# dachinzo/ringpop-node

Measured on AMD Instinct MI355X. Metric: ring lookups/s + member-updates merged/s; SWIM round time @100k members, higher is better.
Workload: dtype u32; 1 GPU; C2: 10000-server HashRing x 100 replica points, batched lookupN(n=3) of 36-byte keys, 2^26 keys per step; servers=10000, replica_points=100, total_keys=164550934528, parallelism=keys sharded, ring replicated

## Files before the change

ringpop-node_amd/csrc/rp_ring.hip:

```cpp
#include <algorithm>
#include <chrono>
#include <cstdio>
#include <cstdlib>
#include <cstring>
#include <memory>
#include <mutex>
#include <string>
#include <unordered_map>
#include <vector>

#include "../../include/ringpop_amd.h"
#include "rp_farmhash.h"
#include "rp_philox.h"
#include "rp_hashlong.h"
#include "rp_names.h"
#include "rp_prims.h"

namespace rp {

constexpr uint32_t NIL = 0xFFFFFFFFu;

static bool getenv_flag(const char* name) {
    const char* v = getenv(name);
    return v && *v && *v != '0';
// ... 620 lines not shown

#ifdef RP_LK_PROF
__device__ unsigned long long g_lk_prof[10];
#define LK_T(var, dep) \
    uint64_t var;      \
    asm volatile("s_memtime %0\n\ts_waitcnt lgkmcnt(0)" : "=s"(var) : "v"(dep))
#else
#define LK_T(var, dep)
#endif

#ifdef RP_LK_ABLATE
#define RP_LKA(cv) ((cv).ablate)
#else
#define RP_LKA(cv) 0u
#endif
template <int KPL, int NEED, int HS = 1, bool FUSE = false, int STG = 0, int LH = 1>
__global__ __launch_bounds__(kLkThreads) __attribute__((amdgpu_waves_per_eu(4))) void k_lookupn_lean(const uint8_t* __restrict__ keys, uint64_t ntiles,
                                                             CompactView cv, uint32_t* __restrict__ out,
                                                             uint8_t* __restrict__ counts,
                                                             uint32_t* __restrict__ slow_list,
                                                             uint32_t* __restrict__ slow_cnt, CompactFixView fv,
                                                             int np) {
    constexpr int LEN = 36, W4 = LEN / 4;
    constexpr int TK = kLkThreads * KPL;
    constexpr int V4 = TK * W4 / 4;
    constexpr int PER = (V4 + kLkThreads - 1) / kLkThreads;
    constexpr int NW = kLkThreads / 64;
    constexpr uint32_t SPAN = 5 - NEED;
    static_assert((TK * W4) % 4 == 0 && (TK * NEED) % 4 == 0 && NEED >= 1 && NEED <= 4, "tile shape");
    static_assert(KPL % HS == 0 && V4 % HS == 0, "slices of whole keys");
    constexpr int SK = TK * W4 / HS, SO = TK * NEED;
    constexpr int VS = V4 / HS;
    constexpr int SKR = STG ? 2 * SK : SK;
    static_assert(STG == 0 || (SK * 4) % 1024 == 0, "DMA slices of whole 1-KB wave pieces");
    __shared__ __attribute__((aligned(16))) uint32_t lds[SKR > SO ? SKR : SO];
    constexpr uint32_t AG = 64;
    __shared__ uint32_t ag[NW][3][AG];
    __shared__ uint32_t nslow_tile;
    uint32_t* const sk = lds;
    uint32_t* const so = lds;
    const int tid = threadIdx.x, lane = tid & 63, wv = tid >> 6;
    const uint32_t omask = (1u << cv.ob) - 1u, obit = 1u << cv.ob;
    const uint32_t bsh = 32u - cv.cb;
    const uint32_t rmask = (1u << bsh) - 1u;
    const __amdgpu_buffer_rsrc_t ent_r =
        __builtin_amdgcn_make_buffer_rsrc(const_cast<uint8_t*>(cv.ent), 0, (int)cv.ent_bytes, 0x00020000);
    const bool hinted = NEED == 3 && cv.idxh != nullptr && !(RP_LKA(cv) & 4u);
    const __amdgpu_buffer_rsrc_t idx_r = __builtin_amdgcn_make_buffer_rsrc(
        const_cast<uint32_t*>(hinted ? cv.idxh : cv.idx), 0, (int)cv.idx_bytes, 0x00020000);
    auto load16 = [&](uint32_t pos) {
        return __builtin_bit_cast(u32x4, __builtin_amdgcn_raw_buffer_load_b128(ent_r, (int)(3u * pos), 0, 0));
    };
    auto ent5v = [&](const u32x4 v, uint32_t (&e)[5]) {
        e[0] = v.x & 0xFFFFFFu;
        e[1] = (v.x >> 24) | ((v.y & 0xFFFFu) << 8);
        e[2] = (v.y >> 16) | ((v.z & 0xFFu) << 16);
        e[3] = v.z >> 8;
        e[4] = v.w & 0xFFFFFFu;
    };
    auto wstart = [&](uint32_t hk, uint32_t bck, uint32_t hint) -> uint32_t {
        const int fl = (int)((((hk << cv.cb) >> 24) * bck) >> 8) - 2 + (int)hint;
        return (NEED >= 2 && cv.wpred && bck <= 10u && fl > 0) ? (uint32_t)fl : 0u;
    };
    auto finish2 = [&](const u32x4 win, uint32_t K, uint32_t w2, uint32_t* row, uint8_t* cnt, uint32_t* nsl,
                       uint32_t* slist) {
        const uint32_t kk = w2 & 0xFFFu, bck = (w2 >> 12) & 15u, b0 = (w2 >> 17) & 15u;
        uint32_t e2[5];
        ent5v(win, e2);
        uint32_t off = 0;
        bool slow = false;
        if ((w2 >> 16) & 1u) {
            bool tie = false;
#pragma unroll
            for (int j = 0; j < 5; j++) {
                const bool inb = (uint32_t)j + b0 < bck;
                off += (inb && e2[j] < K);
                tie |= (inb && e2[j] - K < obit);
            }
            slow = (tie && !cv.exact) | (off == 5u && bck > b0 + 5u) | (((w2 >> 21) & 1u) && off == 0u);
        }
        uint32_t res[4] = {NIL, NIL, NIL, NIL};
        const uint32_t rc = dedupe5(e2, off, omask, NEED, res);
        slow |= rc < (uint32_t)NEED;
        if (slow) {
            const uint32_t sp = atomicAdd(nsl, 1u);
            if (sp < kSlowPerTile) slist[sp] = kk;
        }
#pragma unroll
        for (int q = 0; q < NEED; q++) row[kk * NEED + q] = res[q];
        if (cnt) cnt[kk] = (uint8_t)rc;
    };
#ifdef RP_LK_PROF
    uint64_t pa[6] = {0, 0, 0, 0, 0, 0}, ntl = 0;
#endif
    for (uint64_t t = blockIdx.x; t < ntiles; t += gridDim.x) {
        const uint64_t base = t * TK;
        uint32_t h[KPL];
        LK_T(t0, tid);
        if constexpr (STG == 1 || STG == 2) {
            constexpr int SLB = SK * 4, SLI = SLB / 1024, PW = SLI / NW, PX = SLI % NW;
            const uint8_t* src = keys + base * LEN;
            uint8_t* ring = reinterpret_cast<uint8_t*>(lds);
            auto dma = [&](int sl) {
#pragma unroll
                for (int i = 0; i < PW + 1; i++)
                    if (i < PW || wv < PX) {
// ... 40 lines not shown
#pragma unroll
                for (int k = hs * (KPL / HS); k < (hs + 1) * (KPL / HS); k++) {
                    uint32_t w[W4];
#pragma unroll
                    for (int j = 0; j < W4; j++) w[j] = sb[(tid + (k - hs * (KPL / HS)) * kLkThreads) * W4 + j];
                    h[k] = fh::hash32_words<LEN>(w);
                }
                if (hs + 2 < HS) {
                    asm volatile("s_waitcnt lgkmcnt(0)" ::: "memory");
                    __builtin_amdgcn_s_barrier();
                    asm volatile("" ::: "memory");
                    dma(hs + 2);
                }
            }
        } else {
            const u32x4* s4 = reinterpret_cast<const u32x4*>(keys + base * LEN);
            u32x4 pre[PER];
#pragma unroll
            for (int q = 0; q < PER; q++) {
                const int k = tid + q * kLkThreads;
                if (k < V4) pre[q] = __builtin_nontemporal_load(s4 + k);
            }
            if (tid == 0) nslow_tile = 0;
#pragma unroll
            for (int hs = 0; hs < HS; hs++) {
                if (hs) __syncthreads();
#pragma unroll
                for (int q = 0; q < PER; q++) {
                    const int k = tid + q * kLkThreads;
                    if (k >= hs * VS && k < (hs + 1) * VS) reinterpret_cast<u32x4*>(sk)[k - hs * VS] = pre[q];
                }
                __syncthreads();
#ifdef RP_LK_PROF
                if (hs == 0) {
                    LK_T(tk, sk[tid]);
                    pa[0] += tk - t0;
                }
#endif
#pragma unroll
                for (int k = hs * (KPL / HS); k < (hs + 1) * (KPL / HS); k++) {
                    uint32_t w[W4];
#pragma unroll
                    for (int j = 0; j < W4; j++) w[j] = sk[(tid + (k - hs * (KPL / HS)) * kLkThreads) * W4 + j];
                    h[k] = fh::hash32_words<LEN>(w);
                }
            }
        }
        LK_T(t2, h[KPL - 1]);
        __syncthreads();
        uint32_t nag = 0;
        constexpr int KH = KPL / LH;
        static_assert(KPL % LH == 0, "whole halves");
#ifdef RP_LK_PROF
        uint64_t t3 = 0;
#endif
#pragma unroll
        for (int hh = 0; hh < LH; hh++) {
        if (hh) __builtin_amdgcn_sched_barrier(0);
        u32x2 rec[KH];
#pragma unroll
        for (int kq = 0; kq < KH; kq++) {
            const int k = hh * KH + kq;
            if (RP_LKA(cv) & 4u)
                rec[kq] = u32x2{(uint32_t)(((uint64_t)h[k] * (cv.M - 32u)) >> 32), h[k] & 0x11111111u};
            else
                rec[kq] = __builtin_bit_cast(u32x2, __builtin_amdgcn_raw_buffer_load_b64(idx_r, (int)((h[k] >> (bsh + 3u)) * 8u), 0, 0));
        }
        uint32_t lo[KH], bc[KH], ws[KH];
        u32x4 win[KH];
#pragma unroll
        for (int kq = 0; kq < KH; kq++) {
            const int k = hh * KH + kq;
            const uint32_t s4 = ((h[k] >> bsh) & 7u) * 4u;
            const uint32_t below = rec[kq].y & ((1u << s4) - 1u);
            uint32_t base = rec[kq].x, hint = 1u;
            if (hinted) {
                const uint32_t g = h[k] >> (bsh + 3u);
                base = (uint32_t)(((uint64_t)g * cv.M) >> (cv.cb - 3u)) + (uint32_t)((int32_t)(rec[kq].x << 18) >> 18);
                hint = (rec[kq].x >> (14u + (s4 >> 1))) & 3u;
            }
            lo[kq] = base + __builtin_amdgcn_sad_u8(below & 0x0F0F0F0Fu, 0u,
                                                    __builtin_amdgcn_sad_u8((below >> 4) & 0x0F0F0F0Fu, 0u, 0u));
            bc[kq] = (rec[kq].y >> s4) & 15u;
            ws[kq] = wstart(h[k], bc[kq], hint);
            if (RP_LKA(cv) & 26u) {
                const uint32_t pos = lo[kq] + ws[kq];
                win[kq] = (RP_LKA(cv) & 8u) ? u32x4{rec[kq].x, rec[kq].y, h[k], pos}
                                           : __builtin_bit_cast(u32x4, __builtin_amdgcn_raw_buffer_load_b128(
                                                                          ent_r, (int)((3u * pos) & ((RP_LKA(cv) & 2u) ? ~15u : ~3u)), 0, 0));
            } else {
                win[kq] = load16(lo[kq] + ws[kq]);
            }
        }
#ifdef RP_LK_PROF
        if (hh == 0) {
            LK_T(t3h, lo[KH - 1]);
            t3 = t3h;
        }
#endif
#pragma unroll
        for (int kq = 0; kq < KH; kq++) {
            const int k = hh * KH + kq;
            uint32_t e[5];
            ent5v(win[kq], e);
            const uint32_t K = ((h[k] & rmask) >> cv.fsh) << cv.ob;
            const uint32_t w = ws[kq];
            uint32_t lt = 0;
            bool tie = false;
#pragma unroll
            for (int j = 0; j < 5; j++) {
                const bool inb = (uint32_t)j + w < bc[kq];
                lt += (inb && e[j] < K);
                tie |= (inb && e[j] - K < obit);
            }
            uint32_t r[NEED];
#pragma unroll
            for (int q = 0; q < NEED; q++) {
                uint32_t v = e[q] & omask;
#pragma unroll
                for (uint32_t d = 1; d <= SPAN; d++) v = lt == d ? (e[q + d] & omask) : v;
                r[q] = v;
            }
            bool dup = false;
#pragma unroll
            for (int a = 0; a < NEED; a++)
#pragma unroll
                for (int b = a + 1; b < NEED; b++) dup |= r[a] == r[b];
            const uint32_t kk = tid + k * kLkThreads;
            bool slow = (tie && !cv.exact) | (lo[kq] + 20u > cv.M);
            const bool under = w > 0u && lt == 0u;
            const bool again = !slow && (lt > SPAN || dup || under) && !(RP_LKA(cv) & 1u);
            const uint64_t m = __ballot(again);
            const uint32_t pos = nag + __builtin_amdgcn_mbcnt_hi((uint32_t)(m >> 32), __builtin_amdgcn_mbcnt_lo((uint32_t)m, 0u));
            nag += (uint32_t)__popcll(m);
            if (again) {
                if (pos < AG) {
                    const uint32_t b0 = under ? (w > 2u ? w - 2u : 0u) : w + 5u;
                    const bool search = under || (lt == 5u && bc[kq] > w + 5u);
                    ag[wv][0][pos] = lo[kq] + (search ? b0 : w + lt);
                    ag[wv][1][pos] = K;
                    ag[wv][2][pos] = kk | (bc[kq] << 12) | ((uint32_t)search << 16) | ((search ? b0 : 0u) << 17) |
                                     ((uint32_t)(under && b0 > 0u) << 21);
                } else {
                    slow = true;
                }
            } else {
#pragma unroll
                for (int q = 0; q < NEED; q++) so[kk * NEED + q] = r[q];
                if (counts) counts[base + kk] = (uint8_t)NEED;
            }
            if (slow) {
                const uint32_t sp = atomicAdd(&nslow_tile, 1u);
                if (sp < kSlowPerTile) slow_list[t * kSlowPerTile + sp] = kk;
            }
        }
        }
        LK_T(t4, nag);
        __builtin_amdgcn_fence(__ATOMIC_SEQ_CST, "wavefront");
        for (uint32_t j = lane; j < (nag < AG ? nag : AG); j += 64)
            finish2(load16(ag[wv][0][j]), ag[wv][1][j], ag[wv][2][j], so, counts ? counts + base : nullptr,
                    &nslow_tile, slow_list + t * kSlowPerTile);
        LK_T(t5a, nag);
        __syncthreads();
        LK_T(t5, tid);
        if (tid == 0) slow_cnt[t] = nslow_tile;
        u32x4* d4 = reinterpret_cast<u32x4*>(out + base * NEED);
        const u32x4* s4 = reinterpret_cast<const u32x4*>(so);
#pragma unroll
        for (int k = tid; k < TK * NEED / 4; k += kLkThreads) __builtin_nontemporal_store(s4[k], d4 + k);
        __syncthreads();
#ifdef RP_LK_PROF
        LK_T(t6, tid);
        pa[1] += t2 - t0;
        pa[2] += t3 - t2;
        pa[3] += t4 - t3;
        pa[4] += t5a - t4;
// ... 13 lines not shown
        const uint64_t nt = ntiles > blockIdx.x ? (ntiles - blockIdx.x + gridDim.x - 1) / gridDim.x : 0;
        for (uint64_t i0 = 0; i0 < nt; i0 += TPP) {
            const uint64_t i = i0 + (uint32_t)tid / kSlowPerTile;
            const uint32_t q = (uint32_t)tid % kSlowPerTile;
            if (i < nt) {
                const uint64_t t = blockIdx.x + i * gridDim.x;
                const uint32_t c = slow_cnt[t];
                if (c <= kSlowPerTile) {
                    if (q < c) lookupn_redo(keys, fv, np, (uint32_t)NEED, out, counts, t * TK + slow_list[t * kSlowPerTile + q]);
                } else {
                    for (uint32_t k = q; k < (uint32_t)TK; k += kSlowPerTile) lookupn_redo(keys, fv, np, (uint32_t)NEED, out, counts, t * TK + k);
                }
            }
        }
    }
}

constexpr int kWsSlots = 2;
constexpr uint32_t kWsSpin = 1u << 22;
typedef uint32_t u32x3v __attribute__((ext_vector_type(3)));

template <int NP, int NC, int ABL = 0>
__global__ __launch_bounds__((NP + NC) * 64) __attribute__((amdgpu_waves_per_eu(4))) void k_lookupn_ws(const uint8_t* __restrict__ keys, uint64_t nwt,
                                                               CompactView cv, uint32_t* __restrict__ out,
                                                               uint32_t out_bytes, uint8_t* __restrict__ counts,
                                                               uint32_t* __restrict__ slow_list,
                                                               uint32_t* __restrict__ slow_cnt,
                                                               uint32_t* __restrict__ err) {
    constexpr int NEED = 3, KPL = 8, LEN = 36, W4 = LEN / 4;
    constexpr int TK = 64 * KPL;
// ... 1629 lines not shown
                uint64_t tot = 0, over = 0;
                for (uint64_t t = 0; t < nwt; t++) {
                    tot += c[t];
                    over += c[t] > kSlowPerTile;
                }
                fprintf(stderr, "[rp] ws lookupN %d:%d: %llu keys, %llu deferred, %llu overflowed wave-tiles, err %u\n", wnp,
                        wnc, (unsigned long long)done, (unsigned long long)tot, (unsigned long long)over, c[nwt + 1]);
            }
            if (done < n)
                launch_lookupn_view(r.view(), keys + done * 36, nullptr, 36, nullptr, n - done, np, W, out + done * W,
                                    counts ? counts + done : nullptr, st);
            return;
        }
        int kpl = getenv("RP_LOOKUP_KPL") ? atoi(getenv("RP_LOOKUP_KPL")) : (need == 3 ? 8 : 4);
        if (kpl != 1 && kpl != 2 && !((kpl == 3 || kpl == 8) && need == 3)) kpl = 4;
        if (n < (uint64_t)kLkThreads * kpl) kpl = 4;
        const uint64_t TK = (uint64_t)kLkThreads * kpl;
        const uint64_t ntiles = n / TK, done = ntiles * TK;
        r.slow.reserve(ntiles * kSlowPerTile + 1);
        r.nslow.reserve(ntiles + 1);
        const bool lean = !(getenv("RP_LOOKUP_LEAN") && !strcmp(getenv("RP_LOOKUP_LEAN"), "0"));
        const unsigned g = grid_for(ntiles, 1, (unsigned)env_pos("RP_LOOKUP_GRID", lean ? 4096u : 2048u));
        const int half = getenv("RP_LOOKUP_HALF") ? atoi(getenv("RP_LOOKUP_HALF")) : (kpl == 8 ? 4 : 0);
        const CompactFixView fv{r.tok.p, r.own.p, r.cidx.p, r.view(), r.M, r.ccb};
        const bool fuse = getenv_flag("RP_LOOKUP_FUSEFIX") && lean && half == 4 && kpl == 8 && need == 3 && cv.ablate != 3;
        const bool stg1 = getenv("RP_LOOKUP_STG") && atoi(getenv("RP_LOOKUP_STG")) == 1 && lean && half == 4 && kpl == 8 &&
                          need == 3 && !fuse;
        const bool stg2 = lean && kpl == 8 && need == 3 && !fuse && getenv("RP_LOOKUP_STG") && atoi(getenv("RP_LOOKUP_STG")) == 2;
        const int lh = (lean && (half == 4 || stg2) && kpl == 8 && need == 3 && !fuse)
                           ? (int)env_pos("RP_LOOKUP_LH", stg2 ? 2 : 1) : 1;
        const int stghs = (int)env_pos("RP_LOOKUP_STGHS", 8);
#define RP_COMPACT(KPL, NEED)                                                                                  \
    do {                                                                                                        \
        if (KPL == 8 && NEED == 3 && stg2 && stghs == 8 && lh == 1)                                             \
            hipLaunchKernelGGL((k_lookupn_lean<8, 3, 8, false, 2, 1>), dim3(g), dim3(kLkThreads), 0, st, keys,  \
                               ntiles, cv, out, counts, r.slow.p, r.nslow.p, fv, np);                           \
        else if (KPL == 8 && NEED == 3 && stg2 && stghs == 8)                                                   \
            hipLaunchKernelGGL((k_lookupn_lean<8, 3, 8, false, 2, 2>), dim3(g), dim3(kLkThreads), 0, st, keys,  \
                               ntiles, cv, out, counts, r.slow.p, r.nslow.p, fv, np);                           \
        else if (KPL == 8 && NEED == 3 && stg2)                                                                 \
            hipLaunchKernelGGL((k_lookupn_lean<8, 3, 4, false, 2, 2>), dim3(g), dim3(kLkThreads), 0, st, keys,  \
                               ntiles, cv, out, counts, r.slow.p, r.nslow.p, fv, np);                           \
        else if (KPL == 8 && NEED == 3 && stg1 && lh == 2)                                                      \
            hipLaunchKernelGGL((k_lookupn_lean<8, 3, 4, false, 1, 2>), dim3(g), dim3(kLkThreads), 0, st, keys,  \
                               ntiles, cv, out, counts, r.slow.p, r.nslow.p, fv, np);                           \
        else if (KPL == 8 && NEED == 3 && lh == 2)                                                              \
            hipLaunchKernelGGL((k_lookupn_lean<8, 3, 4, false, 0, 2>), dim3(g), dim3(kLkThreads), 0, st, keys,  \
                               ntiles, cv, out, counts, r.slow.p, r.nslow.p, fv, np);                           \
        else if (KPL == 8 && NEED == 3 && stg1)                                                                 \
            hipLaunchKernelGGL((k_lookupn_lean<8, 3, 4, false, 1>), dim3(g), dim3(kLkThreads), 0, st, keys,     \
                               ntiles, cv, out, counts, r.slow.p, r.nslow.p, fv, np);                           \
        else if (lean && half == 4 && KPL % 4 == 0 && fuse)                                                     \
            hipLaunchKernelGGL((k_lookupn_lean<KPL, NEED, (KPL % 4 == 0 ? 4 : 1), true>), dim3(g), dim3(kLkThreads), \
                               0, st, keys, ntiles, cv, out, counts, r.slow.p, r.nslow.p, fv, np);               \
        else if (lean && half == 4 && KPL % 4 == 0)                                                             \
            hipLaunchKernelGGL((k_lookupn_lean<KPL, NEED, (KPL % 4 == 0 ? 4 : 1)>), dim3(g), dim3(kLkThreads), 0, \
                               st, keys, ntiles, cv, out, counts, r.slow.p, r.nslow.p, fv, np);                  \
        else if (lean && half == 2 && KPL % 2 == 0)                                                             \
            hipLaunchKernelGGL((k_lookupn_lean<KPL, NEED, (KPL % 2 == 0 ? 2 : 1)>), dim3(g), dim3(kLkThreads), 0, \
                               st, keys, ntiles, cv, out, counts, r.slow.p, r.nslow.p, fv, np);                  \
        else if (lean)                                                                                          \
            hipLaunchKernelGGL((k_lookupn_lean<KPL, NEED>), dim3(g), dim3(kLkThreads), 0, st, keys, ntiles, cv,  \
                               out, counts, r.slow.p, r.nslow.p, fv, np);                                       \
        else                                                                                                    \
            hipLaunchKernelGGL((k_lookupn_compact<KPL, NEED>), dim3(g), dim3(kLkThreads), 0, st, keys, ntiles,   \
                               cv, out, counts, r.slow.p, r.nslow.p);                                           \
    } while (0)
#define RP_COMPACT_N(KPL)         \
    switch (need) {               \
        case 1: RP_COMPACT(KPL, 1); break; \
        case 2: RP_COMPACT(KPL, 2); break; \
        case 3: RP_COMPACT(KPL, 3); break; \
        default: RP_COMPACT(KPL, 4); break; \
    }
        if (kpl == 1) {
            RP_COMPACT_N(1);
        } else if (kpl == 2) {
            RP_COMPACT_N(2);
        } else if (kpl == 8 && need == 3) {
            RP_COMPACT(8, 3);
        } else if (kpl == 3 && need == 3) {
            RP_COMPACT(3, 3);


        } else {
            RP_COMPACT_N(4);
        }
#undef RP_COMPACT_N
#undef RP_COMPACT
        const uint64_t fthreads = ntiles * kSlowPerTile;
        if (cv.ablate != 3 && !fuse)
            hipLaunchKernelGGL((k_lookupn_fix_tiles<CompactFixView>), dim3((unsigned)((fthreads + 255) / 256)),
                               dim3(256), 0, st, keys, fv, np, W, out, counts, r.slow.p, r.nslow.p, ntiles,
                               (uint32_t)TK);
        RP_HIP(hipGetLastError());
#ifdef RP_LK_PROF
        if (getenv_flag("RP_LK_PROF_PRINT")) {
            unsigned long long v[10];
            RP_HIP(hipStreamSynchronize(st));
            RP_HIP(hipMemcpyFromSymbol(v, HIP_SYMBOL(g_lk_prof), sizeof v));
            const double nw = (double)(v[6] ? v[6] : 1);
            fprintf(stderr,
                    "[rp] lean phase cycles per wave-tile (%llu): keys-arrive %.0f hash-all %.0f idx %.0f win1+loop %.0f "
                    "finish2 %.0f barrier+store %.0f\n",
                    v[6], v[0] / nw, v[1] / nw, v[2] / nw, v[3] / nw, v[4] / nw, v[5] / nw);
            memset(v, 0, sizeof v);
            RP_HIP(hipMemcpyToSymbol(HIP_SYMBOL(g_lk_prof), v, sizeof v));
        }
#endif
        if (getenv_flag("RP_LOOKUP_DEBUG")) {
            std::vector<uint32_t> c(ntiles);
            RP_HIP(hipMemcpyAsync(c.data(), r.nslow.p, 4 * ntiles, hipMemcpyDeviceToHost, st));
            RP_HIP(hipStreamSynchronize(st));
            uint64_t tot = 0, over = 0;
            for (uint32_t x : c) {
                tot += x;
                over += x > kSlowPerTile;
            }
            fprintf(stderr, "[rp] compact lookupN: %llu keys, %llu deferred, %llu overflowed tiles (cb %u ob %u fsh %u)\n",
                    (unsigned long long)done, (unsigned long long)tot, (unsigned long long)over, r.ccb, r.cob, r.cfsh);
        }
        if (done < n)
            launch_lookupn_view(r.view(), keys + done * 36, nullptr, 36, nullptr, n - done, np, W, out + done * W,
                                counts ? counts + done : nullptr, st);
        return;
    }
    if (use_packed && fixed36 && W <= 4 && need <= 4 && !getenv_flag("RP_RING_NOWINDOW")) {
        RP_REQUIRE(n < (1ull << 32), "lookupn: at most 2^32-1 keys per call");
        r.slow.reserve(n + 1);
        r.nslow.reserve(1);
        RP_HIP(hipMemsetAsync(r.nslow.p, 0, sizeof(uint32_t), st));
        const int ablate = getenv("RP_LOOKUP_ABLATE") ? atoi(getenv("RP_LOOKUP_ABLATE")) : 0;
        const int kpl = getenv("RP_LOOKUP_KPL") ? atoi(getenv("RP_LOOKUP_KPL")) : kDefaultKPL;
        const PackedView pv = r.pview();
#define RP_PROBE(KPL, MODE)                                                                                     \
// ... 2428 lines not shown
```

Before: 76.20 billion lookupN(3)/s.

## Factor lookup stages into reusable helpers and add optional sorted-tile lookup path

```diff
diff --git a/ringpop-node_amd/csrc/rp_ring.hip b/ringpop-node_amd/csrc/rp_ring.hip
--- a/ringpop-node_amd/csrc/rp_ring.hip
+++ b/ringpop-node_amd/csrc/rp_ring.hip
@@ -658,6 +658,189 @@
 #else
 #define RP_LKA(cv) 0u
 #endif
+constexpr uint32_t kLkAG = 64;
+
+template <int NEED, int KB>
+struct LkStages {
+    static constexpr uint32_t SPAN = 5 - NEED;
+    const CompactView& cv;
+    const uint32_t omask, obit, bsh, rmask;
+    const __amdgpu_buffer_rsrc_t ent_r;
+    const bool hinted;
+    const __amdgpu_buffer_rsrc_t idx_r;
+
+    __device__ __forceinline__ explicit LkStages(const CompactView& v)
+        : cv(v), omask((1u << v.ob) - 1u), obit(1u << v.ob), bsh(32u - v.cb), rmask((1u << (32u - v.cb)) - 1u),
+          ent_r(__builtin_amdgcn_make_buffer_rsrc(const_cast<uint8_t*>(v.ent), 0, (int)v.ent_bytes, 0x00020000)),
+          hinted(NEED == 3 && v.idxh != nullptr && !(RP_LKA(v) & 4u)),
+          idx_r(__builtin_amdgcn_make_buffer_rsrc(const_cast<uint32_t*>(hinted ? v.idxh : v.idx), 0,
+                                                  (int)v.idx_bytes, 0x00020000)) {}
+
+    __device__ __forceinline__ u32x4 load16(uint32_t pos) const {
+        return __builtin_bit_cast(u32x4, __builtin_amdgcn_raw_buffer_load_b128(ent_r, (int)(3u * pos), 0, 0));
+    }
+    static __device__ __forceinline__ void ent5v(const u32x4 v, uint32_t (&e)[5]) {
+        e[0] = v.x & 0xFFFFFFu;
+        e[1] = (v.x >> 24) | ((v.y & 0xFFFFu) << 8);
+        e[2] = (v.y >> 16) | ((v.z & 0xFFu) << 16);
+        e[3] = v.z >> 8;
+        e[4] = v.w & 0xFFFFFFu;
+    }
+    __device__ __forceinline__ uint32_t wstart(uint32_t hk, uint32_t bck, uint32_t hint) const {
+        const int fl = (int)((((hk << cv.cb) >> 24) * bck) >> 8) - 2 + (int)hint;
+        return (NEED >= 2 && cv.wpred && bck <= 10u && fl > 0) ? (uint32_t)fl : 0u;
+    }
+    __device__ __forceinline__ u32x2 index_rec(uint32_t hk) const {
+        if (RP_LKA(cv) & 4u)
+            return u32x2{(uint32_t)(((uint64_t)hk * (cv.M - 32u)) >> 32), hk & 0x11111111u};
+        return __builtin_bit_cast(u32x2, __builtin_amdgcn_raw_buffer_load_b64(idx_r, (int)((hk >> (bsh + 3u)) * 8u), 0, 0));
+    }
+    __device__ __forceinline__ u32x4 window(uint32_t hk, const u32x2 rec, uint32_t& lo, uint32_t& bc, uint32_t& ws) const {
+        const uint32_t s4 = ((hk >> bsh) & 7u) * 4u;
+        const uint32_t below = rec.y & ((1u << s4) - 1u);
+        uint32_t base = rec.x, hint = 1u;
+        if (hinted) {
+            const uint32_t g = hk >> (bsh + 3u);
+            base = (uint32_t)(((uint64_t)g * cv.M) >> (cv.cb - 3u)) + (uint32_t)((int32_t)(rec.x << 18) >> 18);
+            hint = (rec.x >> (14u + (s4 >> 1))) & 3u;
+        }
+        lo = base + __builtin_amdgcn_sad_u8(below & 0x0F0F0F0Fu, 0u,
+                                            __builtin_amdgcn_sad_u8((below >> 4) & 0x0F0F0F0Fu, 0u, 0u));
+        bc = (rec.y >> s4) & 15u;
+        ws = wstart(hk, bc, hint);
+        if (RP_LKA(cv) & 26u) {
+            const uint32_t pos = lo + ws;
+            return (RP_LKA(cv) & 8u) ? u32x4{rec.x, rec.y, hk, pos}
+                                     : __builtin_bit_cast(u32x4, __builtin_amdgcn_raw_buffer_load_b128(
+                                                                    ent_r, (int)((3u * pos) & ((RP_LKA(cv) & 2u) ? ~15u : ~3u)), 0, 0));
+        }
+        return load16(lo + ws);
+    }
+    template <class Defer>
+    __device__ __forceinline__ void resolve(const u32x4 win, uint32_t hk, uint32_t lo, uint32_t bc, uint32_t w,
+                                            uint32_t kk, uint32_t& nag, uint32_t (*agw)[kLkAG], uint32_t* so,
+                                            uint8_t* cnt, Defer&& defer) const {
+        uint32_t e[5];
+        ent5v(win, e);
+        const uint32_t K = ((hk & rmask) >> cv.fsh) << cv.ob;
+        uint32_t lt = 0;
+        bool tie = false;
+#pragma unroll
+        for (int j = 0; j < 5; j++) {
+            const bool inb = (uint32_t)j + w < bc;
+            lt += (inb && e[j] < K);
+            tie |= (inb && e[j] - K < obit);
+        }
+        uint32_t r[NEED];
+#pragma unroll
+        for (int q = 0; q < NEED; q++) {
+            uint32_t v = e[q] & omask;
+#pragma unroll
+            for (uint32_t d = 1; d <= SPAN; d++) v = lt == d ? (e[q + d] & omask) : v;
+            r[q] = v;
+        }
+        bool dup = false;
+#pragma unroll
+        for (int a = 0; a < NEED; a++)
+#pragma unroll
+            for (int b = a + 1; b < NEED; b++) dup |= r[a] == r[b];
+        bool slow = (tie && !cv.exact) | (lo + 20u > cv.M);
+        const bool under = w > 0u && lt == 0u;
+        const bool again = !slow && (lt > SPAN || dup || under) && !(RP_LKA(cv) & 1u);
+        const uint64_t m = __ballot(again);
+        const uint32_t pos = nag + __builtin_amdgcn_mbcnt_hi((uint32_t)(m >> 32), __builtin_amdgcn_mbcnt_lo((uint32_t)m, 0u));
+        nag += (uint32_t)__popcll(m);
+        if (again) {
+            if (pos < kLkAG) {
+                const uint32_t b0 = under ? (w > 2u ? w - 2u : 0u) : w + 5u;
+                const bool search = under || (lt == 5u && bc > w + 5u);
+                agw[0][pos] = lo + (search ? b0 : w + lt);
+                agw[1][pos] = K;
+                agw[2][pos] = kk | (bc << KB) | ((uint32_t)search << (KB + 4)) | ((search ? b0 : 0u) << (KB + 5)) |
+                              ((uint32_t)(under && b0 > 0u) << (KB + 9));
+            } else {
+                slow = true;
+            }
+        } else {
+#pragma unroll
+            for (int q = 0; q < NEED; q++) so[kk * NEED + q] = r[q];
+            if (cnt) cnt[kk] = (uint8_t)NEED;
+        }
+        if (slow) defer(kk);
+    }
+    template <class Defer>
+    __device__ __forceinline__ void finish2(const u32x4 win, uint32_t K, uint32_t w2, uint32_t* row, uint8_t* cnt,
+                                            Defer&& defer) const {
+        const uint32_t kk = w2 & ((1u << KB) - 1u), bck = (w2 >> KB) & 15u, b0 = (w2 >> (KB + 5)) & 15u;
+        uint32_t e2[5];
+        ent5v(win, e2);
+        uint32_t off = 0;
+        bool slow = false;
+        if ((w2 >> (KB + 4)) & 1u) {
+            bool tie = false;
+#pragma unroll
+            for (int j = 0; j < 5; j++) {
+                const bool inb = (uint32_t)j + b0 < bck;
+                off += (inb && e2[j] < K);
+                tie |= (inb && e2[j] - K < obit);
+            }
+            slow = (tie && !cv.exact) | (off == 5u && bck > b0 + 5u) | (((w2 >> (KB + 9)) & 1u) && off == 0u);
+        }
+        uint32_t res[4] = {NIL, NIL, NIL, NIL};
+        const uint32_t rc = dedupe5(e2, off, omask, NEED, res);
+        slow |= rc < (uint32_t)NEED;
+        if (slow) defer(kk);
+#pragma unroll
+        for (int q = 0; q < NEED; q++) row[kk * NEED + q] = res[q];
+        if (cnt) cnt[kk] = (uint8_t)rc;
+    }
+};
+
+template <int THREADS, int KPL, int HS, bool WAVE = false, class Issued, class Arrived>
+__device__ __forceinline__ void lk_key_stage(const uint8_t* __restrict__ tile_keys, uint32_t* sk, int tid,
+                                             uint32_t (&h)[KPL], Issued&& issued, Arrived&& arrived) {
+    constexpr int LEN = 36, W4 = LEN / 4;
+    constexpr int V4 = THREADS * KPL * W4 / 4;
+    constexpr int PER = (V4 + THREADS - 1) / THREADS;
+    constexpr int VS = V4 / HS;
+    static_assert(KPL % HS == 0 && V4 % HS == 0, "slices of whole keys");
+    const u32x4* s4 = reinterpret_cast<const u32x4*>(tile_keys);
+    u32x4 pre[PER];
+#pragma unroll
+    for (int q = 0; q < PER; q++) {
+        const int k = tid + q * THREADS;
+        if (k < V4) pre[q] = __builtin_nontemporal_load(s4 + k);
+    }
+    static_assert(!WAVE || THREADS == 64, "a wave's own tile");
+    auto meet = [] {
+        if constexpr (WAVE) {
+            __builtin_amdgcn_fence(__ATOMIC_SEQ_CST, "wavefront");
+            __builtin_amdgcn_wave_barrier();
+        } else {
+            __syncthreads();
+        }
+    };
+    issued();
+#pragma unroll
+    for (int hs = 0; hs < HS; hs++) {
+        if (hs) meet();
+#pragma unroll
+        for (int q = 0; q < PER; q++) {
+            const int k = tid + q * THREADS;
+            if (k >= hs * VS && k < (hs + 1) * VS) reinterpret_cast<u32x4*>(sk)[k - hs * VS] = pre[q];
+        }
+        meet();
+        if (hs == 0) arrived();
+#pragma unroll
+        for (int k = hs * (KPL / HS); k < (hs + 1) * (KPL / HS); k++) {
+            uint32_t w[W4];
+#pragma unroll
+            for (int j = 0; j < W4; j++) w[j] = sk[(tid + (k - hs * (KPL / HS)) * THREADS) * W4 + j];
+            h[k] = fh::hash32_words<LEN>(w);
+        }
+    }
+}
+
 template <int KPL, int NEED, int HS = 1, bool FUSE = false, int STG = 0, int LH = 1>
 __global__ __launch_bounds__(kLkThreads) __attribute__((amdgpu_waves_per_eu(4))) void k_lookupn_lean(const uint8_t* __restrict__ keys, uint64_t ntiles,
                                                              CompactView cv, uint32_t* __restrict__ out,
@@ -668,72 +851,21 @@
     constexpr int LEN = 36, W4 = LEN / 4;
     constexpr int TK = kLkThreads * KPL;
     constexpr int V4 = TK * W4 / 4;
-    constexpr int PER = (V4 + kLkThreads - 1) / kLkThreads;
     constexpr int NW = kLkThreads / 64;
-    constexpr uint32_t SPAN = 5 - NEED;
     static_assert((TK * W4) % 4 == 0 && (TK * NEED) % 4 == 0 && NEED >= 1 && NEED <= 4, "tile shape");
     static_assert(KPL % HS == 0 && V4 % HS == 0, "slices of whole keys");
     constexpr int SK = TK * W4 / HS, SO = TK * NEED;
-    constexpr int VS = V4 / HS;
     constexpr int SKR = STG ? 2 * SK : SK;
     static_assert(STG == 0 || (SK * 4) % 1024 == 0, "DMA slices of whole 1-KB wave pieces");
     __shared__ __attribute__((aligned(16))) uint32_t lds[SKR > SO ? SKR : SO];
-    constexpr uint32_t AG = 64;
+    constexpr uint32_t AG = kLkAG;
     __shared__ uint32_t ag[NW][3][AG];
     __shared__ uint32_t nslow_tile;
     uint32_t* const sk = lds;
     uint32_t* const so = lds;
     const int tid = threadIdx.x, lane = tid & 63, wv = tid >> 6;
-    const uint32_t omask = (1u << cv.ob) - 1u, obit = 1u << cv.ob;
-    const uint32_t bsh = 32u - cv.cb;
-    const uint32_t rmask = (1u << bsh) - 1u;
-    const __amdgpu_buffer_rsrc_t ent_r =
-        __builtin_amdgcn_make_buffer_rsrc(const_cast<uint8_t*>(cv.ent), 0, (int)cv.ent_bytes, 0x00020000);
-    const bool hinted = NEED == 3 && cv.idxh != nullptr && !(RP_LKA(cv) & 4u);
-    const __amdgpu_buffer_rsrc_t idx_r = __builtin_amdgcn_make_buffer_rsrc(
-        const_cast<uint32_t*>(hinted ? cv.idxh : cv.idx), 0, (int)cv.idx_bytes, 0x00020000);
-    auto load16 = [&](uint32_t pos) {
-        return __builtin_bit_cast(u32x4, __builtin_amdgcn_raw_buffer_load_b128(ent_r, (int)(3u * pos), 0, 0));
-    };
-    auto ent5v = [&](const u32x4 v, uint32_t (&e)[5]) {
-        e[0] = v.x & 0xFFFFFFu;
-        e[1] = (v.x >> 24) | ((v.y & 0xFFFFu) << 8);
-        e[2] = (v.y >> 16) | ((v.z & 0xFFu) << 16);
-        e[3] = v.z >> 8;
-        e[4] = v.w & 0xFFFFFFu;
-    };
-    auto wstart = [&](uint32_t hk, uint32_t bck, uint32_t hint) -> uint32_t {
-        const int fl = (int)((((hk << cv.cb) >> 24) * bck) >> 8) - 2 + (int)hint;
-        return (NEED >= 2 && cv.wpred && bck <= 10u && fl > 0) ? (uint32_t)fl : 0u;
-    };
-    auto finish2 = [&](const u32x4 win, uint32_t K, uint32_t w2, uint32_t* row, uint8_t* cnt, uint32_t* nsl,
-                       uint32_t* slist) {
-        const uint32_t kk = w2 & 0xFFFu, bck = (w2 >> 12) & 15u, b0 = (w2 >> 17) & 15u;
-        uint32_t e2[5];
-        ent5v(win, e2);
-        uint32_t off = 0;
-        bool slow = false;
-        if ((w2 >> 16) & 1u) {
-            bool tie = false;
-#pragma unroll
-            for (int j = 0; j < 5; j++) {
-                const bool inb = (uint32_t)j + b0 < bck;
-                off += (inb && e2[j] < K);
-                tie |= (inb && e2[j] - K < obit);
-            }
-            slow = (tie && !cv.exact) | (off == 5u && bck > b0 + 5u) | (((w2 >> 21) & 1u) && off == 0u);
-        }
-        uint32_t res[4] = {NIL, NIL, NIL, NIL};
-        const uint32_t rc = dedupe5(e2, off, omask, NEED, res);
-        slow |= rc < (uint32_t)NEED;
-        if (slow) {
-            const uint32_t sp = atomicAdd(nsl, 1u);
-            if (sp < kSlowPerTile) slist[sp] = kk;
-        }
-#pragma unroll
-        for (int q = 0; q < NEED; q++) row[kk * NEED + q] = res[q];
-        if (cnt) cnt[kk] = (uint8_t)rc;
-    };
+    const LkStages<NEED, 12> lk(cv);
+    static_assert(TK <= (1 << 12), "a tile slot is 12 bits of a list word");
 #ifdef RP_LK_PROF
     uint64_t pa[6] = {0, 0, 0, 0, 0, 0}, ntl = 0;
 #endif
@@ -804,41 +936,23 @@
                 }
             }
         } else {
-            const u32x4* s4 = reinterpret_cast<const u32x4*>(keys + base * LEN);
-            u32x4 pre[PER];
-#pragma unroll
-            for (int q = 0; q < PER; q++) {
-                const int k = tid + q * kLkThreads;
-                if (k < V4) pre[q] = __builtin_nontemporal_load(s4 + k);
-            }
-            if (tid == 0) nslow_tile = 0;
-#pragma unroll
-            for (int hs = 0; hs < HS; hs++) {
-                if (hs) __syncthreads();
-#pragma unroll
-                for (int q = 0; q < PER; q++) {
-                    const int k = tid + q * kLkThreads;
-                    if (k >= hs * VS && k < (hs + 1) * VS) reinterpret_cast<u32x4*>(sk)[k - hs * VS] = pre[q];
-                }
-                __syncthreads();
+            lk_key_stage<kLkThreads, KPL, HS>(
+                keys + base * LEN, sk, tid, h, [&] { if (tid == 0) nslow_tile = 0; },
+                [&] {
 #ifdef RP_LK_PROF
-                if (hs == 0) {
                     LK_T(tk, sk[tid]);
                     pa[0] += tk - t0;
-                }
 #endif
-#pragma unroll
-                for (int k = hs * (KPL / HS); k < (hs + 1) * (KPL / HS); k++) {
-                    uint32_t w[W4];
-#pragma unroll
-                    for (int j = 0; j < W4; j++) w[j] = sk[(tid + (k - hs * (KPL / HS)) * kLkThreads) * W4 + j];
-                    h[k] = fh::hash32_words<LEN>(w);
-                }
-            }
+                });
         }
         LK_T(t2, h[KPL - 1]);
         __syncthreads();
         uint32_t nag = 0;
+        uint8_t* const cnt_tile = counts ? counts + base : nullptr;
+        auto defer = [&](uint32_t kk) {
+            const uint32_t sp = atomicAdd(&nslow_tile, 1u);
+            if (sp < kSlowPerTile) slow_list[t * kSlowPerTile + sp] = kk;
+        };
         constexpr int KH = KPL / LH;
         static_assert(KPL % LH == 0, "whole halves");
 #ifdef RP_LK_PROF
@@ -849,39 +963,11 @@
         if (hh) __builtin_amdgcn_sched_barrier(0);
         u32x2 rec[KH];
 #pragma unroll
-        for (int kq = 0; kq < KH; kq++) {
-            const int k = hh * KH + kq;
-            if (RP_LKA(cv) & 4u)
-                rec[kq] = u32x2{(uint32_t)(((uint64_t)h[k] * (cv.M - 32u)) >> 32), h[k] & 0x11111111u};
-            else
-                rec[kq] = __builtin_bit_cast(u32x2, __builtin_amdgcn_raw_buffer_load_b64(idx_r, (int)((h[k] >> (bsh + 3u)) * 8u), 0, 0));
-        }
+        for (int kq = 0; kq < KH; kq++) rec[kq] = lk.index_rec(h[hh * KH + kq]);
         uint32_t lo[KH], bc[KH], ws[KH];
         u32x4 win[KH];
 #pragma unroll
-        for (int kq = 0; kq < KH; kq++) {
-            const int k = hh * KH + kq;
-            const uint32_t s4 = ((h[k] >> bsh) & 7u) * 4u;
-            const uint32_t below = rec[kq].y & ((1u << s4) - 1u);
-            uint32_t base = rec[kq].x, hint = 1u;
-            if (hinted) {
-                const uint32_t g = h[k] >> (bsh + 3u);
-                base = (uint32_t)(((uint64_t)g * cv.M) >> (cv.cb - 3u)) + (uint32_t)((int32_t)(rec[kq].x << 18) >> 18);
-                hint = (rec[kq].x >> (14u + (s4 >> 1))) & 3u;
-            }
-            lo[kq] = base + __builtin_amdgcn_sad_u8(below & 0x0F0F0F0Fu, 0u,
-                                                    __builtin_amdgcn_sad_u8((below >> 4) & 0x0F0F0F0Fu, 0u, 0u));
-            bc[kq] = (rec[kq].y >> s4) & 15u;
-            ws[kq] = wstart(h[k], bc[kq], hint);
-            if (RP_LKA(cv) & 26u) {
-                const uint32_t pos = lo[kq] + ws[kq];
-                win[kq] = (RP_LKA(cv) & 8u) ? u32x4{rec[kq].x, rec[kq].y, h[k], pos}
-                                           : __builtin_bit_cast(u32x4, __builtin_amdgcn_raw_buffer_load_b128(
-                                                                          ent_r, (int)((3u * pos) & ((RP_LKA(cv) & 2u) ? ~15u : ~3u)), 0, 0));
-            } else {
-                win[kq] = load16(lo[kq] + ws[kq]);
-            }
-        }
+        for (int kq = 0; kq < KH; kq++) win[kq] = lk.window(h[hh * KH + kq], rec[kq], lo[kq], bc[kq], ws[kq]);
 #ifdef RP_LK_PROF
         if (hh == 0) {
             LK_T(t3h, lo[KH - 1]);
@@ -891,65 +977,14 @@
 #pragma unroll
         for (int kq = 0; kq < KH; kq++) {
             const int k = hh * KH + kq;
-            uint32_t e[5];
-            ent5v(win[kq], e);
-            const uint32_t K = ((h[k] & rmask) >> cv.fsh) << cv.ob;
-            const uint32_t w = ws[kq];
-            uint32_t lt = 0;
-            bool tie = false;
-#pragma unroll
-            for (int j = 0; j < 5; j++) {
-                const bool inb = (uint32_t)j + w < bc[kq];
-                lt += (inb && e[j] < K);
-                tie |= (inb && e[j] - K < obit);
-            }
-            uint32_t r[NEED];
-#pragma unroll
-            for (int q = 0; q < NEED; q++) {
-                uint32_t v = e[q] & omask;
-#pragma unroll
-                for (uint32_t d = 1; d <= SPAN; d++) v = lt == d ? (e[q + d] & omask) : v;
-                r[q] = v;
-            }
-            bool dup = false;
-#pragma unroll
-            for (int a = 0; a < NEED; a++)
-#pragma unroll
-                for (int b = a + 1; b < NEED; b++) dup |= r[a] == r[b];
-            const uint32_t kk = tid + k * kLkThreads;
-            bool slow = (tie && !cv.exact) | (lo[kq] + 20u > cv.M);
-            const bool under = w > 0u && lt == 0u;
-            const bool again = !slow && (lt > SPAN || dup || under) && !(RP_LKA(cv) & 1u);
-            const uint64_t m = __ballot(again);
-            const uint32_t pos = nag + __builtin_amdgcn_mbcnt_hi((uint32_t)(m >> 32), __builtin_amdgcn_mbcnt_lo((uint32_t)m, 0u));
-            nag += (uint32_t)__popcll(m);
-            if (again) {
-                if (pos < AG) {
-                    const uint32_t b0 = under ? (w > 2u ? w - 2u : 0u) : w + 5u;
-                    const bool search = under || (lt == 5u && bc[kq] > w + 5u);
-                    ag[wv][0][pos] = lo[kq] + (search ? b0 : w + lt);
-                    ag[wv][1][pos] = K;
-                    ag[wv][2][pos] = kk | (bc[kq] << 12) | ((uint32_t)search << 16) | ((search ? b0 : 0u) << 17) |
-                                     ((uint32_t)(under && b0 > 0u) << 21);
-                } else {
-                    slow = true;
-                }
-            } else {
-#pragma unroll
-                for (int q = 0; q < NEED; q++) so[kk * NEED + q] = r[q];
-                if (counts) counts[base + kk] = (uint8_t)NEED;
-            }
-            if (slow) {
-                const uint32_t sp = atomicAdd(&nslow_tile, 1u);
-                if (sp < kSlowPerTile) slow_list[t * kSlowPerTile + sp] = kk;
-            }
+            lk.resolve(win[kq], h[k], lo[kq], bc[kq], ws[kq], (uint32_t)(tid + k * kLkThreads), nag, ag[wv], so, cnt_tile,
+                       defer);
         }
         }
         LK_T(t4, nag);
         __builtin_amdgcn_fence(__ATOMIC_SEQ_CST, "wavefront");
         for (uint32_t j = lane; j < (nag < AG ? nag : AG); j += 64)
-            finish2(load16(ag[wv][0][j]), ag[wv][1][j], ag[wv][2][j], so, counts ? counts + base : nullptr,
-                    &nslow_tile, slow_list + t * kSlowPerTile);
+            lk.finish2(lk.load16(ag[wv][0][j]), ag[wv][1][j], ag[wv][2][j], so, cnt_tile, defer);
         LK_T(t5a, nag);
         __syncthreads();
         LK_T(t5, tid);
@@ -993,6 +1028,141 @@
             }
         }
     }
+}
+
+#ifdef RP_LK_PROF
+__device__ unsigned long long g_sk_prof[10];
+#endif
+constexpr int kSortDefault = 256;
+
+template <int THREADS, int NEED>
+__global__ __launch_bounds__(THREADS) __attribute__((amdgpu_waves_per_eu(4))) void k_lookupn_sorted(
+    const uint8_t* __restrict__ keys, uint64_t ntiles, CompactView cv, uint32_t* __restrict__ out,
+    uint8_t* __restrict__ counts, uint32_t* __restrict__ slow_list, uint32_t* __restrict__ slow_cnt) {
+    constexpr int LEN = 36, W4 = LEN / 4, KPL = 8, HS = 4;
+    constexpr int TK = THREADS * KPL;
+    constexpr int NW = THREADS / 64;
+    constexpr int SUB = TK / 2048;
+    constexpr int SK = TK * W4 / HS, SO = TK * NEED;
+    constexpr int BINS = THREADS;
+    constexpr int BSH = 32 - (BINS == 256 ? 8 : BINS == 512 ? 9 : 10);
+    constexpr int CW = BINS / 2;
+    constexpr int WPL = CW / 64;
+    static_assert(THREADS == 256 || THREADS == 512 || THREADS == 1024, "whole 2,048-key logical tiles, 13-bit slots, 16-bit bin counters");
+    static_assert(2 * TK <= SO && SK <= SO, "the ordered pairs and the key slice fit under the rows");
+    __shared__ __attribute__((aligned(16))) uint32_t lds[SO];
+    __shared__ uint32_t ag[NW][3][kLkAG];
+    __shared__ uint32_t bins[CW];
+    __shared__ uint32_t nslow_sub[SUB];
+    uint32_t* const sk = lds;
+    uint32_t* const so = lds;
+    u32x2* const pairs = reinterpret_cast<u32x2*>(lds);
+    const int tid = threadIdx.x, lane = tid & 63, wv = tid >> 6;
+    const LkStages<NEED, 13> lk(cv);
+#ifdef RP_LK_PROF
+    uint64_t pa[6] = {0, 0, 0, 0, 0, 0}, ntl = 0;
+#endif
+    if (tid < CW) bins[tid] = 0;
+    if (tid < SUB) nslow_sub[tid] = 0;
+    for (uint64_t t = blockIdx.x; t < ntiles; t += gridDim.x) {
+        const uint64_t base = t * TK;
+        uint32_t h[KPL], kk[KPL];
+        LK_T(t0, tid);
+        lk_key_stage<64, KPL, HS, true>(keys + (base + (uint64_t)wv * 512) * LEN, sk + wv * (SK / NW), lane, h, [] {}, [] {});
+        LK_T(t1, h[KPL - 1]);
+        uint32_t rank[KPL];
+#pragma unroll
+        for (int k = 0; k < KPL; k++) {
+            const uint32_t b = h[k] >> BSH, sh = (b & 1u) * 16u;
+            rank[k] = (atomicAdd(&bins[b >> 1], 1u << sh) >> sh) & 0xFFFFu;
+        }
+        __syncthreads();
+        if (wv == 0) {
+            uint32_t c[WPL], sum = 0;
+#pragma unroll
+            for (int i = 0; i < WPL; i++) {
+                c[i] = bins[lane * WPL + i];
+                sum += (c[i] & 0xFFFFu) + (c[i] >> 16);
+            }
+            uint32_t x = sum;
+#pragma unroll
+            for (int o = 1; o < 64; o <<= 1) {
+                const uint32_t y = __shfl_up(x, o, 64);
+                if (lane >= o) x += y;
+            }
+            uint32_t run = x - sum;
+#pragma unroll
+            for (int i = 0; i < WPL; i++) {
+                const uint32_t a = run, b = run + (c[i] & 0xFFFFu);
+                run = b + (c[i] >> 16);
+                bins[lane * WPL + i] = a | (b << 16);
+            }
+        }
+        __syncthreads();
+#pragma unroll
+        for (int k = 0; k < KPL; k++) {
+            const uint32_t b = h[k] >> BSH, sh = (b & 1u) * 16u;
+            const uint32_t slot = ((bins[b >> 1] >> sh) & 0xFFFFu) + rank[k];
+            pairs[slot] = u32x2{h[k], (uint32_t)(wv * 512 + lane + 64 * k)};
+        }
+        __syncthreads();
+#pragma unroll
+        for (int k = 0; k < KPL; k++) {
+            const u32x2 p = pairs[tid + k * THREADS];
+            h[k] = p.x;
+            kk[k] = p.y;
+        }
+        if (tid < CW) bins[tid] = 0;
+        if (tid < SUB) nslow_sub[tid] = 0;
+        LK_T(t2, kk[KPL - 1]);
+        __syncthreads();
+        uint32_t nag = 0;
+        uint8_t* const cnt_tile = counts ? counts + base : nullptr;
+        auto defer = [&](uint32_t k) {
+            const uint32_t s = k >> 11;
+            const uint32_t sp = atomicAdd(&nslow_sub[s], 1u);
+            if (sp < kSlowPerTile) slow_list[(t * SUB + s) * kSlowPerTile + sp] = k & 2047u;
+        };
+        u32x2 rec[KPL];
+#pragma unroll
+        for (int k = 0; k < KPL; k++) rec[k] = lk.index_rec(h[k]);
+        uint32_t lo[KPL], bc[KPL], ws[KPL];
+        u32x4 win[KPL];
+#pragma unroll
+        for (int k = 0; k < KPL; k++) win[k] = lk.window(h[k], rec[k], lo[k], bc[k], ws[k]);
+        LK_T(t3, lo[KPL - 1]);
+#pragma unroll
+        for (int k = 0; k < KPL; k++) lk.resolve(win[k], h[k], lo[k], bc[k], ws[k], kk[k], nag, ag[wv], so, cnt_tile, defer);
+        LK_T(t4, nag);
+        __builtin_amdgcn_fence(__ATOMIC_SEQ_CST, "wavefront");
+        for (uint32_t j = lane; j < (nag < kLkAG ? nag : kLkAG); j += 64)
+            lk.finish2(lk.load16(ag[wv][0][j]), ag[wv][1][j], ag[wv][2][j], so, cnt_tile, defer);
+        LK_T(t5a, nag);
+        __syncthreads();
+        LK_T(t5, tid);
+        if (tid < SUB) slow_cnt[t * SUB + tid] = nslow_sub[tid];
+        u32x4* d4 = reinterpret_cast<u32x4*>(out + base * NEED);
+        const u32x4* s4 = reinterpret_cast<const u32x4*>(so);
+#pragma unroll
+        for (int k = tid; k < TK * NEED / 4; k += THREADS) __builtin_nontemporal_store(s4[k], d4 + k);
+        __syncthreads();
+#ifdef RP_LK_PROF
+        LK_T(t6, tid);
+        pa[0] += t1 - t0;
+        pa[1] += t2 - t1;
+        pa[2] += t3 - t2;
+        pa[3] += t4 - t3;
+        pa[4] += t5a - t4;
+        pa[5] += t6 - t5;
+        ntl += 1;
+#endif
+    }
+#ifdef RP_LK_PROF
+    if (lane == 0) {
+        for (int i = 0; i < 6; i++) atomicAdd(&g_sk_prof[i], (unsigned long long)pa[i]);
+        atomicAdd(&g_sk_prof[6], (unsigned long long)ntl);
+    }
+#endif
 }
 
 constexpr int kWsSlots = 2;
@@ -2652,11 +2822,39 @@
         }
         int kpl = getenv("RP_LOOKUP_KPL") ? atoi(getenv("RP_LOOKUP_KPL")) : (need == 3 ? 8 : 4);
         if (kpl != 1 && kpl != 2 && !((kpl == 3 || kpl == 8) && need == 3)) kpl = 4;
-        if (n < (uint64_t)kLkThreads * kpl) kpl = 4;
+        int sort_t = kSortDefault;
+        if (const char* e = getenv("RP_LOOKUP_SORT")) sort_t = atoi(e);
+        RP_REQUIRE(sort_t == 0 || sort_t == 256 || sort_t == 512 || sort_t == 1024, "RP_LOOKUP_SORT: one of 0, 256, 512, 1024");
+        if (need != 3 || !cv.idxh || cv.ablate != 0 || n < 8ull * (uint64_t)sort_t || getenv("RP_LOOKUP_KPL") ||
+            getenv("RP_LOOKUP_HALF") || getenv("RP_LOOKUP_LEAN") || getenv("RP_LOOKUP_STG") || getenv("RP_LOOKUP_LH") ||
+            getenv_flag("RP_LOOKUP_FUSEFIX"))
+            sort_t = 0;
+        const uint64_t stiles = sort_t ? n / (8ull * (uint64_t)sort_t) : 0;
+        const uint64_t s0 = stiles * 8ull * (uint64_t)sort_t;
+        const uint64_t t0 = s0 / 2048;
+        if (!sort_t && n < (uint64_t)kLkThreads * kpl) kpl = 4;
         const uint64_t TK = (uint64_t)kLkThreads * kpl;
-        const uint64_t ntiles = n / TK, done = ntiles * TK;
-        r.slow.reserve(ntiles * kSlowPerTile + 1);
-        r.nslow.reserve(ntiles + 1);
+        const uint64_t ntiles = (n - s0) / TK, done = s0 + ntiles * TK;
+        r.slow.reserve((t0 + ntiles) * kSlowPerTile + 1);
+        r.nslow.reserve(t0 + ntiles + 1);
+        const uint8_t* const lkeys = keys + s0 * 36;
+        uint32_t* const lout = out + s0 * W;
+        uint8_t* const lcounts = counts ? counts + s0 : nullptr;
+        uint32_t* const lslow = r.slow.p + t0 * kSlowPerTile;
+        uint32_t* const lnslow = r.nslow.p + t0;
+        if (stiles) {
+            const unsigned sg = grid_for(stiles, 1, (unsigned)env_pos("RP_LOOKUP_GRID", sort_t == 256 ? 4096u : sort_t == 512 ? 8192u : 1024u));
+#define RP_SORTED(T) \
+    hipLaunchKernelGGL((k_lookupn_sorted<T, 3>), dim3(sg), dim3(T), 0, st, keys, stiles, cv, out, counts, r.slow.p, r.nslow.p)
+            if (sort_t == 256)
+                RP_SORTED(256);
+            else if (sort_t == 512)
+                RP_SORTED(512);
+            else
+                RP_SORTED(1024);
+#undef RP_SORTED
+            RP_HIP(hipGetLastError());
+        }
         const bool lean = !(getenv("RP_LOOKUP_LEAN") && !strcmp(getenv("RP_LOOKUP_LEAN"), "0"));
         const unsigned g = grid_for(ntiles, 1, (unsigned)env_pos("RP_LOOKUP_GRID", lean ? 4096u : 2048u));
         const int half = getenv("RP_LOOKUP_HALF") ? atoi(getenv("RP_LOOKUP_HALF")) : (kpl == 8 ? 4 : 0);
@@ -2671,38 +2869,38 @@
 #define RP_COMPACT(KPL, NEED)                                                                                  \
     do {                                                                                                        \
         if (KPL == 8 && NEED == 3 && stg2 && stghs == 8 && lh == 1)                                             \
-            hipLaunchKernelGGL((k_lookupn_lean<8, 3, 8, false, 2, 1>), dim3(g), dim3(kLkThreads), 0, st, keys,  \
-                               ntiles, cv, out, counts, r.slow.p, r.nslow.p, fv, np);                           \
+            hipLaunchKernelGGL((k_lookupn_lean<8, 3, 8, false, 2, 1>), dim3(g), dim3(kLkThreads), 0, st, lkeys, \
+                               ntiles, cv, lout, lcounts, lslow, lnslow, fv, np);                             \
         else if (KPL == 8 && NEED == 3 && stg2 && stghs == 8)                                                   \
-            hipLaunchKernelGGL((k_lookupn_lean<8, 3, 8, false, 2, 2>), dim3(g), dim3(kLkThreads), 0, st, keys,  \
-                               ntiles, cv, out, counts, r.slow.p, r.nslow.p, fv, np);                           \
+            hipLaunchKernelGGL((k_lookupn_lean<8, 3, 8, false, 2, 2>), dim3(g), dim3(kLkThreads), 0, st, lkeys, \
+                               ntiles, cv, lout, lcounts, lslow, lnslow, fv, np);                             \
         else if (KPL == 8 && NEED == 3 && stg2)                                                                 \
-            hipLaunchKernelGGL((k_lookupn_lean<8, 3, 4, false, 2, 2>), dim3(g), dim3(kLkThreads), 0, st, keys,  \
-                               ntiles, cv, out, counts, r.slow.p, r.nslow.p, fv, np);                           \
+            hipLaunchKernelGGL((k_lookupn_lean<8, 3, 4, false, 2, 2>), dim3(g), dim3(kLkThreads), 0, st, lkeys, \
+                               ntiles, cv, lout, lcounts, lslow, lnslow, fv, np);                             \
         else if (KPL == 8 && NEED == 3 && stg1 && lh == 2)                                                      \
-            hipLaunchKernelGGL((k_lookupn_lean<8, 3, 4, false, 1, 2>), dim3(g), dim3(kLkThreads), 0, st, keys,  \
-                               ntiles, cv, out, counts, r.slow.p, r.nslow.p, fv, np);                           \
+            hipLaunchKernelGGL((k_lookupn_lean<8, 3, 4, false, 1, 2>), dim3(g), dim3(kLkThreads), 0, st, lkeys, \
+                               ntiles, cv, lout, lcounts, lslow, lnslow, fv, np);                             \
         else if (KPL == 8 && NEED == 3 && lh == 2)                                                              \
-            hipLaunchKernelGGL((k_lookupn_lean<8, 3, 4, false, 0, 2>), dim3(g), dim3(kLkThreads), 0, st, keys,  \
-                               ntiles, cv, out, counts, r.slow.p, r.nslow.p, fv, np);                           \
+            hipLaunchKernelGGL((k_lookupn_lean<8, 3, 4, false, 0, 2>), dim3(g), dim3(kLkThreads), 0, st, lkeys, \
+                               ntiles, cv, lout, lcounts, lslow, lnslow, fv, np);                             \
         else if (KPL == 8 && NEED == 3 && stg1)                                                                 \
-            hipLaunchKernelGGL((k_lookupn_lean<8, 3, 4, false, 1>), dim3(g), dim3(kLkThreads), 0, st, keys,     \
-                               ntiles, cv, out, counts, r.slow.p, r.nslow.p, fv, np);                           \
+            hipLaunchKernelGGL((k_lookupn_lean<8, 3, 4, false, 1>), dim3(g), dim3(kLkThreads), 0, st, lkeys,    \
+                               ntiles, cv, lout, lcounts, lslow, lnslow, fv, np);                             \
         else if (lean && half == 4 && KPL % 4 == 0 && fuse)                                                     \
             hipLaunchKernelGGL((k_lookupn_lean<KPL, NEED, (KPL % 4 == 0 ? 4 : 1), true>), dim3(g), dim3(kLkThreads), \
-                               0, st, keys, ntiles, cv, out, counts, r.slow.p, r.nslow.p, fv, np);               \
+                               0, st, lkeys, ntiles, cv, lout, lcounts, lslow, lnslow, fv, np);               \
         else if (lean && half == 4 && KPL % 4 == 0)                                                             \
             hipLaunchKernelGGL((k_lookupn_lean<KPL, NEED, (KPL % 4 == 0 ? 4 : 1)>), dim3(g), dim3(kLkThreads), 0, \
-                               st, keys, ntiles, cv, out, counts, r.slow.p, r.nslow.p, fv, np);                  \
+                               st, lkeys, ntiles, cv, lout, lcounts, lslow, lnslow, fv, np);                  \
         else if (lean && half == 2 && KPL % 2 == 0)                                                             \
             hipLaunchKernelGGL((k_lookupn_lean<KPL, NEED, (KPL % 2 == 0 ? 2 : 1)>), dim3(g), dim3(kLkThreads), 0, \
-                               st, keys, ntiles, cv, out, counts, r.slow.p, r.nslow.p, fv, np);                  \
+                               st, lkeys, ntiles, cv, lout, lcounts, lslow, lnslow, fv, np);                  \
         else if (lean)                                                                                          \
-            hipLaunchKernelGGL((k_lookupn_lean<KPL, NEED>), dim3(g), dim3(kLkThreads), 0, st, keys, ntiles, cv,  \
-                               out, counts, r.slow.p, r.nslow.p, fv, np);                                       \
+            hipLaunchKernelGGL((k_lookupn_lean<KPL, NEED>), dim3(g), dim3(kLkThreads), 0, st, lkeys, ntiles, cv, \
+                               lout, lcounts, lslow, lnslow, fv, np);                                           \
         else                                                                                                    \
-            hipLaunchKernelGGL((k_lookupn_compact<KPL, NEED>), dim3(g), dim3(kLkThreads), 0, st, keys, ntiles,   \
-                               cv, out, counts, r.slow.p, r.nslow.p);                                           \
+            hipLaunchKernelGGL((k_lookupn_compact<KPL, NEED>), dim3(g), dim3(kLkThreads), 0, st, lkeys, ntiles,  \
+                               cv, lout, lcounts, lslow, lnslow);                                               \
     } while (0)
 #define RP_COMPACT_N(KPL)         \
     switch (need) {               \
@@ -2711,7 +2909,8 @@
         case 3: RP_COMPACT(KPL, 3); break; \
         default: RP_COMPACT(KPL, 4); break; \
     }
-        if (kpl == 1) {
+        if (ntiles == 0) {
+        } else if (kpl == 1) {
             RP_COMPACT_N(1);
         } else if (kpl == 2) {
             RP_COMPACT_N(2);
@@ -2726,10 +2925,10 @@
         }
 #undef RP_COMPACT_N
 #undef RP_COMPACT
-        const uint64_t fthreads = ntiles * kSlowPerTile;
+        const uint64_t fthreads = (t0 + ntiles) * kSlowPerTile;
         if (cv.ablate != 3 && !fuse)
             hipLaunchKernelGGL((k_lookupn_fix_tiles<CompactFixView>), dim3((unsigned)((fthreads + 255) / 256)),
-                               dim3(256), 0, st, keys, fv, np, W, out, counts, r.slow.p, r.nslow.p, ntiles,
+                               dim3(256), 0, st, keys, fv, np, W, out, counts, r.slow.p, r.nslow.p, t0 + ntiles,
                                (uint32_t)TK);
         RP_HIP(hipGetLastError());
 #ifdef RP_LK_PROF
@@ -2744,19 +2943,29 @@
                     v[6], v[0] / nw, v[1] / nw, v[2] / nw, v[3] / nw, v[4] / nw, v[5] / nw);
             memset(v, 0, sizeof v);
             RP_HIP(hipMemcpyToSymbol(HIP_SYMBOL(g_lk_prof), v, sizeof v));
+            if (stiles) {
+                RP_HIP(hipMemcpyFromSymbol(v, HIP_SYMBOL(g_sk_prof), sizeof v));
+                const double sw = (double)(v[6] ? v[6] : 1);
+                fprintf(stderr,
+                        "[rp] sorted<%d> phase cycles per wave-tile (%llu): keys+hash %.0f sort+deal %.0f idx+win-issue %.0f "
+                        "win1+loop %.0f finish2 %.0f barrier+store %.0f\n",
+                        sort_t, v[6], v[0] / sw, v[1] / sw, v[2] / sw, v[3] / sw, v[4] / sw, v[5] / sw);
+                memset(v, 0, sizeof v);
+                RP_HIP(hipMemcpyToSymbol(HIP_SYMBOL(g_sk_prof), v, sizeof v));
+            }
         }
 #endif
         if (getenv_flag("RP_LOOKUP_DEBUG")) {
-            std::vector<uint32_t> c(ntiles);
-            RP_HIP(hipMemcpyAsync(c.data(), r.nslow.p, 4 * ntiles, hipMemcpyDeviceToHost, st));
+            std::vector<uint32_t> c(t0 + ntiles);
+            RP_HIP(hipMemcpyAsync(c.data(), r.nslow.p, 4 * (t0 + ntiles), hipMemcpyDeviceToHost, st));
             RP_HIP(hipStreamSynchronize(st));
             uint64_t tot = 0, over = 0;
             for (uint32_t x : c) {
                 tot += x;
                 over += x > kSlowPerTile;
             }
-            fprintf(stderr, "[rp] compact lookupN: %llu keys, %llu deferred, %llu overflowed tiles (cb %u ob %u fsh %u)\n",
-                    (unsigned long long)done, (unsigned long long)tot, (unsigned long long)over, r.ccb, r.cob, r.cfsh);
+            fprintf(stderr, "[rp] compact lookupN: %llu keys, %llu deferred, %llu overflowed tiles (cb %u ob %u fsh %u sort %d)\n",
+                    (unsigned long long)done, (unsigned long long)tot, (unsigned long long)over, r.ccb, r.cob, r.cfsh, sort_t);
         }
         if (done < n)
             launch_lookupn_view(r.view(), keys + done * 36, nullptr, 36, nullptr, n - done, np, W, out + done * W,
```

Result: faster. 79.90 billion lookupN(3)/s (median of 6 runs) (+4.8%).
